# stochasticHydroTools/PSE

Measured on AMD Instinct MI355X. Metric: BD particle-steps/s (full PSE Brownian step: M.F + k-space noise + Lanczos M^1/2.psi + Euler), N=1e6, phi=0.1, higher is better.
Workload: dtype f64; 1 GPU; random-sphere suspension N=1000000, phi=0.1, cubic L=347.29, grid 256^3, xi=0.4405, rcut=5.966, P=6, error=0.001, kT=1.0, dt=0.001; parallelism=1 GPU

## Files before the change

include/pse_amd.h:

```cpp
#ifndef PSE_AMD_H
#define PSE_AMD_H

#ifdef __cplusplus
extern "C" {
#endif

typedef struct { double x, y, z, w; } pse_double4;
typedef struct { double x, y, z; } pse_double3;
typedef struct { int x, y, z; } pse_int3;

typedef struct pse_handle pse_handle;

enum pse_status {
    PSE_OK = 0,
    PSE_ERR_INVALID = -1,
    PSE_ERR_HIP = -2,
    PSE_ERR_FFT = -3,
    PSE_ERR_COMM = -4,
    PSE_ERR_NUMERIC = -5
};

typedef struct pse_params {
    unsigned int n_max;
    double Lx, Ly, Lz, xy;
// ... 241 lines not shown
int pse_angle_forces(pse_angles *a, const pse_double4 *pos, pse_double4 *force ,
                     int accumulate, double *out8 );

#define PSE_DIHEDRAL_HARMONIC 0
#define PSE_DIHEDRAL_OPLS     1
typedef struct pse_dihedrals pse_dihedrals;
int pse_dihedrals_create(pse_handle *h, unsigned n, unsigned ndihedrals,
                         const unsigned *quads_host ,
                         const unsigned *types_host ,
                         int ntypes, const int *kind_host , const double *params_host ,
                         pse_dihedrals **out);
int pse_dihedrals_destroy(pse_dihedrals *d);
int pse_dihedral_forces(pse_dihedrals *d, const pse_double4 *pos, pse_double4 *force ,
                        int accumulate, double *out8 );
int pse_debug_copy_grid(pse_handle *h, int stage, double *host_out);
int pse_debug_spread(pse_handle *h, const pse_double4 *pos, const pse_double4 *force, const unsigned int *group_members,
                     unsigned int N);
int pse_debug_gather(pse_handle *h, const pse_double4 *pos, const double *grid_host, const unsigned int *group_members,
                     unsigned int N, pse_double4 *vel_out);
int pse_debug_far_path(pse_handle *h, unsigned int N, int *out6);
int pse_debug_wave_grid(pse_handle *h, const double *grid_in_host, double xi, double eta, int noise, double kT, double dt,
                        unsigned int timestep, int poison, double *grid_out_host);
int pse_debug_fft_path(pse_handle *h, int *out8);
int pse_debug_kvector(pse_handle *h, int n, const int *ijk_host, double *out_host);
int pse_debug_grid_placement(pse_handle *h, int *tried, float *ms_first, float *ms_kept);
int pse_debug_vq_roundtrip(int n, const double *rows_host, double *out_host);
#define PSE_DEBUG_LZ_NSCAL 400
typedef struct pse_debug_lz_decision {
    int m_lo, m_hi, done_iters, have_last_beta, pending_beta, first, last, normalised, m_max;
    double tol, seq;
} pse_debug_lz_decision;
typedef struct pse_debug_lz_outcome {
    int done, m_final, checked, status;
    double stepnorm;
    double t_prev[104];
    double coef[104];
    double mirror[5];
} pse_debug_lz_outcome;
int pse_debug_lz_decide(const double *scal_host, int n_dec, const pse_debug_lz_decision *dec, double open0, pse_debug_lz_outcome *out);
int pse_debug_lz_decide_supported(int m_hi);
int pse_debug_matvec_ms(pse_handle *h, int reps, float *ms_per_launch);

typedef struct pse_team pse_team;
int pse_team_unique_id(void *id128_host);
int pse_team_create(pse_handle **members, int n_members, const void *id128_host, pse_team **out);
typedef struct pse_host_xfer {
// ... 77 lines not shown
```

pse_amd/_lib.py:

```python
import ctypes
import os

_HERE = os.path.dirname(os.path.abspath(__file__))


def asan_dir():
    d = os.environ.get("PSE_ASAN_DIR")
    if not d:
        return None
    if not os.path.exists(os.path.join(d, ".pse_asan_build")):
        import sys
        print(f"pse_amd: PSE_ASAN_DIR={d} ignored: no sanitizer build there (python -m pse_amd.build --asan writes one)", file=sys.stderr)
        return None
    if not getattr(asan_dir, "_said", False):
        import sys
        print(f"pse_amd: using the CPU SANITIZER build in {d} (PSE_ASAN_DIR): device entry points are stubs", file=sys.stderr)
        asan_dir._said = True
    return d


_ASAN_DIR = asan_dir()
LIB_PATH = os.path.join(_ASAN_DIR or _HERE, "libpse_amd.so")

PSE_OK = 0
# ... 155 lines not shown
    "pse_isf_store": (_i, [_vp, _i]),
    "pse_isf_correlate": (_i, [_vp, _i, _vp, _vp, _i, _vp, _vp]),
    "pse_host_rouse_weights": (_i, [_u, _i, _vp]),
    "pse_bonds_create": (_i, [_vp, _u, _u, _vp, _vp, _i, _vp, _vp, _vp, _vp]),
    "pse_bonds_destroy": (_i, [_vp]),
    "pse_bond_forces": (_i, [_vp, _vp, _vp, _i, _vp]),
    "pse_bonds_overstretched": (_i, [_vp, _vp]),
    "pse_host_bond_rows": (_i, [_u, _u, _vp, _vp, _vp, _vp]),
    "pse_angles_create": (_i, [_vp, _u, _u, _vp, _vp, _i, _vp, _vp, _vp, _vp]),
    "pse_angles_destroy": (_i, [_vp]),
    "pse_angle_forces": (_i, [_vp, _vp, _vp, _i, _vp]),
    "pse_host_angle_rows": (_i, [_u, _u, _vp, _vp, _vp, _vp]),
    "pse_dihedrals_create": (_i, [_vp, _u, _u, _vp, _vp, _i, _vp, _vp, _vp]),
    "pse_dihedrals_destroy": (_i, [_vp]),
    "pse_dihedral_forces": (_i, [_vp, _vp, _vp, _i, _vp]),
    "pse_host_dihedral_rows": (_i, [_u, _u, _vp, _vp, _vp, _vp]),
    "pse_eval_realspace": (_i, [_vp, _dp, _i, _dp, _dp]),
    "pse_debug_copy_grid": (_i, [_vp, _i, _dp]),
    "pse_debug_spread": (_i, [_vp, _vp, _vp, _vp, _u]),
    "pse_debug_gather": (_i, [_vp, _vp, _dp, _vp, _u, _vp]),
    "pse_debug_far_path": (_i, [_vp, _u, _ip]),
    "pse_debug_wave_grid": (_i, [_vp, _dp, _d, _d, _i, _d, _d, _u, _i, _dp]),
    "pse_debug_fft_path": (_i, [_vp, _ip]),
    "pse_debug_kvector": (_i, [_vp, _i, _ip, _dp]),
    "pse_debug_grid_placement": (_i, [_vp, _ip, ctypes.POINTER(ctypes.c_float), ctypes.POINTER(ctypes.c_float)]),
    "pse_debug_vq_roundtrip": (_i, [_i, _dp, _dp]),
    "pse_debug_lz_decide": (_i, [_dp, _i, ctypes.POINTER(pse_debug_lz_decision), _d, ctypes.POINTER(pse_debug_lz_outcome)]),
    "pse_debug_lz_decide_supported": (_i, [_i]),
    "pse_debug_matvec_ms": (_i, [_vp, _i, ctypes.POINTER(ctypes.c_float)]),
    "pse_team_unique_id": (_i, [_vp]),
    "pse_team_create": (_i, [ctypes.POINTER(_vp), _i, _vp, ctypes.POINTER(_vp)]),
    "pse_team_create_transport": (_i, [_vp, ctypes.POINTER(pse_transport), ctypes.POINTER(_vp)]),
    "pse_team_destroy": (_i, [_vp]),
    "pse_team_debug_solo": (_i, [_vp, _i]),
    "pse_team_mobility": (_i, [_vp, ctypes.POINTER(_vp), ctypes.POINTER(_vp), ctypes.POINTER(_vp), _vp, _u, _i]),
    "pse_team_brownian_velocity": (_i, [_vp, ctypes.POINTER(_vp), ctypes.POINTER(_vp), ctypes.POINTER(_vp), _vp, _u, _d, _d, _u, _ip]),
    "pse_team_step": (_i, [_vp, ctypes.POINTER(_vp), ctypes.POINTER(_vp), ctypes.POINTER(_vp), ctypes.POINTER(_vp),
                           ctypes.POINTER(_vp), _vp, _u, _d, _d, _u, _d, _ip]),
    "pse_team_step_local": (_i, [_vp, ctypes.POINTER(_vp), ctypes.POINTER(_vp), ctypes.POINTER(_vp), ctypes.POINTER(_vp),
                                 ctypes.POINTER(_vp), ctypes.POINTER(_vp), ctypes.POINTER(_vp), _d, _d, _u, _d, _i, _ip]),
    "pse_local_layout": (_i, [_vp, _ip, _ip, _ip, _ip, _ip]),
    "pse_team_local_status": (_i, [_vp, _ip]),
    "pse_team_set_lanczos_extra": (_i, [_vp, _i]),
    "pse_set_lanczos_extra": (_i, [_vp, _i]),
    "pse_set_lanczos_operator": (_i, [_vp, _i]),
    "pse_get_lanczos_operator": (_i, [_vp, _ip]),
# ... 41 lines not shown
```

pse_amd/csrc/asan_stub.cpp:

```cpp
#include <algorithm>
#include <cmath>
#include <cstdint>
#include <vector>

#include "pse_err.h"

using namespace pse;

struct Topology;
struct pse_handle {
    pse_params par;
    Derived d;
    pse_info info;
    std::vector<double> coef;
    int n_intervals = 0;
    unsigned long long steps = 0;
    int lz_op = PSE_LANCZOS_RECORDS16;
    std::vector<Topology *> topologies;
};
struct Topology {
    pse_handle *h;
    std::vector<int> row_off;
    std::vector<unsigned> entries;
    Topology(pse_handle *h, size_t noff, size_t nent) : h(h), row_off(noff), entries(nent) {}
// ... 422 lines not shown
    if (!force && !out8) return fail(PSE_ERR_INVALID, "pse_dihedral_forces: force and out8 are both null: nothing to compute");
    return 0;
}

int pse_set_stream(pse_handle *, void *) { return no_device("pse_set_stream"); }
int pse_set_timing(pse_handle *, int) { return no_device("pse_set_timing"); }
int pse_set_async(pse_handle *, int) { return no_device("pse_set_async"); }
int pse_set_timestep_offset(pse_handle *, const unsigned int *) { return no_device("pse_set_timestep_offset"); }
int pse_debug_last_gate(pse_handle *, int *) { return no_device("pse_debug_last_gate"); }
int pse_set_neighbor_skin(pse_handle *, double) { return no_device("pse_set_neighbor_skin"); }
int pse_neighbor_stats(pse_handle *, double *, unsigned long long *, unsigned long long *) { return no_device("pse_neighbor_stats"); }
int pse_mobility(pse_handle *, const pse_double4 *, const pse_double4 *, pse_double4 *, const unsigned int *, unsigned int, int) { return no_device("pse_mobility"); }
int pse_brownian_velocity(pse_handle *, const pse_double4 *, const pse_double4 *, pse_double4 *, const unsigned int *, unsigned int, double,
                          double, unsigned int, int *) { return no_device("pse_brownian_velocity"); }
int pse_sqrt_mreal(pse_handle *, const pse_double4 *, const pse_double4 *, pse_double4 *, const unsigned int *, unsigned int, double, int *) { return no_device("pse_sqrt_mreal"); }
int pse_random_psi(pse_handle *, pse_double4 *, const unsigned int *, unsigned int, unsigned int) { return no_device("pse_random_psi"); }
int pse_eval_realspace(pse_handle *, const double *, int, double *, double *) { return no_device("pse_eval_realspace"); }
int pse_debug_copy_grid(pse_handle *, int, double *) { return no_device("pse_debug_copy_grid"); }
int pse_debug_spread(pse_handle *, const pse_double4 *, const pse_double4 *, const unsigned int *, unsigned int) { return no_device("pse_debug_spread"); }
int pse_debug_gather(pse_handle *, const pse_double4 *, const double *, const unsigned int *, unsigned int, pse_double4 *) { return no_device("pse_debug_gather"); }
int pse_debug_far_path(pse_handle *, unsigned int, int *) { return no_device("pse_debug_far_path"); }
int pse_debug_wave_grid(pse_handle *, const double *, double, double, int, double, double, unsigned int, int, double *) { return no_device("pse_debug_wave_grid"); }
int pse_debug_fft_path(pse_handle *, int *) { return no_device("pse_debug_fft_path"); }
int pse_debug_kvector(pse_handle *, int, const int *, double *) { return no_device("pse_debug_kvector"); }
int pse_debug_grid_placement(pse_handle *, int *, float *, float *) { return no_device("pse_debug_grid_placement"); }
int pse_debug_vq_roundtrip(int, const double *, double *) { return no_device("pse_debug_vq_roundtrip"); }
int pse_debug_lz_decide(const double *, int, const pse_debug_lz_decision *, double, pse_debug_lz_outcome *) { return no_device("pse_debug_lz_decide"); }
int pse_debug_lz_decide_supported(int) { return 0; }
int pse_debug_matvec_ms(pse_handle *, int, float *) { return no_device("pse_debug_matvec_ms"); }
int pse_set_lanczos_extra(pse_handle *, int) { return no_device("pse_set_lanczos_extra"); }
int pse_set_lanczos_operator(pse_handle *h, int op) {
    if (!h) return fail(PSE_ERR_INVALID, "pse_set_lanczos_operator: null handle");
    if (op != PSE_LANCZOS_RECORDS16 && op != PSE_LANCZOS_FP64) return fail(PSE_ERR_INVALID, "pse_set_lanczos_operator: %d is not an operator", op);
    h->lz_op = op;
    return 0;
}
int pse_get_lanczos_operator(pse_handle *h, int *op) {
    if (!h || !op) return fail(PSE_ERR_INVALID, "pse_get_lanczos_operator: null argument");
    *op = h->lz_op;
    return 0;
}
int pse_brownian_velocity_part(pse_handle *, const pse_double4 *, const pse_double4 *, pse_double4 *, const unsigned int *, unsigned int, double,
                               double, unsigned int, int, int *) { return no_device("pse_brownian_velocity_part"); }
int pse_integrate(pse_handle *, pse_double4 *, const pse_double4 *, pse_double3 *, pse_int3 *, const pse_double4 *, const unsigned int *, unsigned int,
                  double, double) { return no_device("pse_integrate"); }
int pse_team_redistribute_local(pse_team *, pse_double4 *const *, pse_double4 *const *, pse_double3 *const *, pse_int3 *const *, pse_double4 *const *,
// ... 21 lines not shown
```

pse_amd/csrc/pse_capi.hip:

```cpp
#include <hip/hip_runtime.h>
#include <rccl/rccl.h>
#include <rocfft/rocfft.h>

#include <algorithm>
#include <chrono>
#include <cmath>
#include <cstdarg>
#include <cstdio>
#include <cstring>
#include <dlfcn.h>
#include <functional>
#include <future>
#include <memory>
#include <mutex>
#include <thread>
#include <string>
#include <vector>

#include "../../include/pse_amd.h"
#include "pse_err.h"
#include "pse_host.h"
#include "pse_kernels.h"
#include "pse_farfield.h"
#include "pse_fft.h"
// ... 791 lines not shown
    const double seq = (double)++h->lz_seq;
    h->lz_last_queued = true;
    int rg[3][2];
    const int nrg_all = update_ranges(h, N, rg);
    VecOut y = lz_y(h, false);
    auto vector_part = [&](int j, const int *gate) {
        launch_lz_update(lz_vec(h, j), y, lz_vec(h, j - 1), lz_vec(h, j + 1), j, h->scal, rg, nrg_all, h->stream,
                         nullptr, 0, h->sc_host_dev, gate, vq_of(h), h->lz_sums);
    };
    auto iteration = [&](int j, bool scalars_only, const int *gate) -> int {
        const bool have_y = j == 0 && h->w_is_mpsi;
        const bool fused = !have_y && h->nb.cap > 0 && h->nb_valid;
        if (!fused && !have_y) {
            if (gate) return fail(PSE_ERR_NUMERIC, "queued Lanczos: a gated iteration needs the pair list");
            TRY(lz_real_ok(h, j));
            TRY(real(T, j == 0 ? &pse_handle::psi_s : &pse_handle::V, &pse_handle::w_s, (size_t)j * h->n_pad, 0, N, true));
        }
        y = lz_y(h, fused);
        const double4 *vjm1 = lz_vec4(h, j - 1);
        const bool split = fused && j > 0;
        if (fused)
            launch_mreal_lanczos(h->pos_s, lz_vec(h, j), y, row_map(0, N), h->cell_off, h->dbox, h->nc, h->d.rcut, h->d.self, h->coef, h->nb,
                                 LzFuse{split ? nullptr : vjm1, h->partials, h->npart_cap, nullptr, nullptr, nullptr, h->lz_sums, lz_update_grid(N)}, h->scal, nullptr, nullptr, h->stream,
                                 h->vl_use ? h->vl : VerletList{}, split ? 4 : 1, gate, DevRowArgs{}, j > 0 ? vq_of(h) : nullptr);
        else if (!(j == 0 && h->sums0_done))
            launch_lz_dots(lz_vec4(h, j), h->w_s, vjm1, 0, N, h->partials, h->npart_cap, h->scal, h->stream);
        h->w_is_mpsi = false; h->sums0_done = false;
        if (scalars_only) launch_lz_update(lz_vec(h, j), y, lz_vec(h, j - 1), lz_vec(h, j + 1), j, h->scal, rg, 0, h->stream, nullptr, 0,
                                           h->sc_host_dev, gate);
        else vector_part(j, gate);
        return 0;
    };
    for (int j = 0; j < target; ++j) TRY(iteration(j, j == target - 1, nullptr));
    LzDecide d{};
    d.m_lo = std::max(m_in - 1, 1); d.m_hi = target; d.done_iters = target; d.first = 1; d.last = extra == 0 ? 1 : 0; d.m_max = M_MAX; d.tol = tol;
    launch_lz_decide(d, h->scal, h->lz_state, h->sc_host_dev, seq, h->stream);
    int done = target;
    for (int x = 0; x < extra; ++x) {
        vector_part(done - 1, stop);
        TRY(iteration(done, true, stop));
        d.m_lo = d.m_hi = done + 1; d.done_iters = done + 1; d.pending_beta = done; d.first = 0; d.last = x == extra - 1 ? 1 : 0;
        launch_lz_decide(d, h->scal, h->lz_state, h->sc_host_dev, seq, h->stream);
        ++done;
    }
    TRY(te(h, PH_LANCZOS));
    if (before_first_wait) TRY(before_first_wait());
    if (before_combine) TRY(before_combine());
// ... 28 lines not shown
                             h == h0 ? h->sc_host_dev : nullptr, nullptr, T.G <= 1 ? vq_of(h) : nullptr, T.G <= 1 ? h->lz_sums : nullptr);
        }
    };
    while (true) {
        for (; done < target; ++done) {
            const bool have_y = done == 0 && h0->w_is_mpsi;
            const bool fused = !have_y && h0->nb.cap > 0 && h0->nb_valid;
            const bool timed = done == 1 && fused;
            if (!fused && !have_y) {
                TRY(lz_real_ok(h0, done));
                TRY(real(T, done == 0 ? &pse_handle::psi_s : &pse_handle::V, &pse_handle::w_s, (size_t)done * h0->n_pad, 0, N, true));
            }
            y_from_list = fused;
            for (pse_handle *h : act(T)) {
                int lo, hi;
                row_range(h, N, lo, hi);
                const double4 *vjm1 = lz_vec4(h, done - 1);
                if (fused) {
                    const bool ev = timed && h->timing;
                    const bool split = done > 0 && T.G <= 1;
                    launch_mreal_lanczos(h->pos_s, lz_vec(h, done), lz_y(h, true), row_map(lo, hi), h->cell_off, h->dbox, h->nc, h->d.rcut, h->d.self, h->coef,
                                         h->nb, LzFuse{split ? nullptr : vjm1, h->partials, h->npart_cap, nullptr, nullptr, nullptr, h->lz_sums, lz_update_grid(N)}, h->scal,
                                         ev ? h->ph[PH_MATVEC].a : nullptr, ev ? h->ph[PH_MATVEC].b : nullptr, h->stream,
                                         h->vl_use ? h->vl : VerletList{}, split ? 4 : 1, nullptr, DevRowArgs{}, done > 0 && T.G <= 1 ? vq_of(h) : nullptr);
                    if (timed) h->matvec_timed = true;
                } else if (!(done == 0 && h->sums0_done)) {
                    launch_lz_dots(lz_vec4(h, done), h->w_s, vjm1, lo, hi, h->partials, h->npart_cap, h->scal, h->stream);
                }
                h->w_is_mpsi = false; h->sums0_done = false;
            }
            if (pump) TRY(pump->upto(n_exchanges));
            ++n_exchanges;
            TRY(team_lanczos_exchange(T, [](pse_handle *h) { return (double *)h->w_s; }));
            update(done, done == target - 1);
        }
        TRY(lz_wait_scalars(T, hook_done, before_first_wait));
        if (T.solo >= 0) { st.m_final = done; break; }
        LzDecide d{};
        d.first = pending_beta == 0; d.pending_beta = pending_beta;
        TRY(lz_decide_batch(d, m_in, done, tol, sc, st));
        if (st.done) break;
        update(done - 1, false);
        pending_beta = done;
        target = std::min(M_MAX, done + std::max(2, done / 4));
    }
    if (st.m_final == 0) {
        if (m_io) *m_io = m_in;
// ... 566 lines not shown
        e = hipStreamSynchronize(h->stream);
    }
    if (e == hipSuccess) e = hipMemcpy(f_host, buf + n, n * sizeof(double), hipMemcpyDeviceToHost);
    if (e == hipSuccess) e = hipMemcpy(g_host, buf + 2 * n, n * sizeof(double), hipMemcpyDeviceToHost);
    (void)hipFree(buf);
    if (e != hipSuccess) return fail(PSE_ERR_HIP, "pse_eval_realspace: %s", hipGetErrorString(e));
    return 0;
}

extern "C" int pse_debug_matvec_ms(pse_handle *h, int reps, float *ms_per_launch) {
    if (!h || !ms_per_launch || reps < 1) return fail(PSE_ERR_INVALID, "pse_debug_matvec_ms: bad argument");
    HIPCHK(hipSetDevice(h->device));
    if (h->n_slabs != 1 || !h->nb_valid || h->nb.cap <= 0 || h->sorted_N <= 0)
        return fail(PSE_ERR_INVALID, "pse_debug_matvec_ms: needs the pair list of a Brownian call on a single-GPU engine (call it right after one)");
    const int N = h->sorted_N;
    RowMap rm{};
    rm.n = 1; rm.lo[0] = 0; rm.hi[0] = N;
    hipEvent_t e0 = nullptr, e1 = nullptr;
    HIPCHK(hipEventCreate(&e0)); HIPCHK(hipEventCreate(&e1));
    auto run = [&](int n) {
        for (int r = 0; r < n; ++r)
            launch_mreal_lanczos(h->pos_s, lz_vec(h, 1), lz_y(h, true), rm, h->cell_off, h->dbox, h->nc, h->d.rcut, h->d.self, h->coef, h->nb,
                                 LzFuse{h->psi_s, h->partials, h->npart_cap, nullptr, nullptr, nullptr}, h->scal, nullptr, nullptr, h->stream,
                                 VerletList{}, 1, nullptr, DevRowArgs{}, vq_of(h), true);
    };
    run(2);
    HIPCHK(hipEventRecord(e0, h->stream));
    run(reps);
    HIPCHK(hipEventRecord(e1, h->stream));
    HIPCHK(hipEventSynchronize(e1));
    float ms = 0;
    HIPCHK(hipEventElapsedTime(&ms, e0, e1));
    (void)hipEventDestroy(e0); (void)hipEventDestroy(e1);
    HIPCHK(hipGetLastError());
    *ms_per_launch = ms / (float)reps;
    return 0;
}
extern "C" int pse_debug_vq_roundtrip(int n, const double *rows_host, double *out_host) {
    if (n < 0 || (n > 0 && (!rows_host || !out_host))) return fail(PSE_ERR_INVALID, "pse_debug_vq_roundtrip: null argument");
    if (n == 0) return 0;
    double *d_in = nullptr, *d_out = nullptr;
    hipError_t e = hipMalloc((void **)&d_in, (size_t)3 * n * sizeof(double));
    if (e == hipSuccess) e = hipMalloc((void **)&d_out, (size_t)3 * n * sizeof(double));
    if (e == hipSuccess) e = hipMemcpy(d_in, rows_host, (size_t)3 * n * sizeof(double), hipMemcpyHostToDevice);
    if (e == hipSuccess) { launch_vq_roundtrip(d_in, d_out, n, nullptr); e = hipGetLastError(); }
    if (e == hipSuccess) e = hipMemcpy(out_host, d_out, (size_t)3 * n * sizeof(double), hipMemcpyDeviceToHost);
    (void)hipFree(d_in); (void)hipFree(d_out);
// ... 123 lines not shown
        if (grid_in_host) HIPCHK(hipMemcpyAsync(dst, grid_in_host + (size_t)c * plane * G.nxl, plane * G.nxl * sizeof(double), hipMemcpyHostToDevice, h->wstream));
        else HIPCHK(hipMemsetAsync(dst, 0, plane * G.nxl * sizeof(double), h->wstream));
    }
    WaveArgs a{0, noise != 0, kT, dt, timestep};
    a.xi = xi; a.eta = eta;
    TRY(wave_forward_transforms(h, 1));
    TRY(wave_compute(T, a, 1));
    TRY(wave_compute(T, a, 2));
    HIPCHK(hipGetLastError());
    HIPCHK(hipStreamSynchronize(h->wstream));
    for (int c = 0; c < 3; ++c)
        HIPCHK(hipMemcpy(grid_out_host + (size_t)c * plane * G.nxl, h->rgrid + c * nr + plane * G.hl, plane * G.nxl * sizeof(double),
                         hipMemcpyDeviceToHost));
    return 0;
}

extern "C" int pse_debug_fft_path(pse_handle *h, int *out8) {
    if (!h || !out8) return fail(PSE_ERR_INVALID, "pse_debug_fft_path: null argument");
    const FftChoice none{FFT_ROCFFT, 0};
    const FftChoice x = h->xfuse ? xfft_choice(h->G, scale_args(h, false, 0.0, 1.0, 0)) : none;
    const FftChoice y = h->own_y ? yfft_choice(h->G, h->tun.yfft_kb) : none;
    const int out[8] = {h->xfuse, h->own_y, h->own_z, x.kernel, x.kb, y.kernel, y.kb, h->own_z ? zfft_choice(h->G.Nz) : FFT_ROCFFT};
    std::copy(out, out + 8, out8);
    return 0;
}

extern "C" int pse_debug_copy_grid(pse_handle *h, int stage, double *host_out) {
    if (!h || !host_out) return fail(PSE_ERR_INVALID, "bad argument");
    (void)stage;
    HIPCHK(hipSetDevice(h->device));
    HIPCHK(hipStreamSynchronize(h->stream));
    if (h->side) HIPCHK(hipStreamSynchronize(h->side));
    const size_t plane = (size_t)h->G.Ny * h->G.Nz, full = plane * (h->G.nxl + h->G.hl + h->G.nhalo);
    for (int c = 0; c < 3; ++c)
        HIPCHK(hipMemcpy(host_out + (size_t)c * plane * h->G.nxl, h->rgrid + c * full + plane * h->G.hl, plane * h->G.nxl * sizeof(double),
                         hipMemcpyDeviceToHost));
    return 0;
}

extern "C" int pse_team_unique_id(void *id128_host) {
    if (!id128_host) return fail(PSE_ERR_INVALID, "null argument");
    static_assert(sizeof(ncclUniqueId) == 128, "RCCL unique id is 128 bytes");
    ncclUniqueId id;
    NCCLCHK(ncclGetUniqueId(&id));
    memcpy(id128_host, &id, sizeof id);
    return 0;
// ... 337 lines not shown
```

pse_amd/csrc/pse_engine.hip:

```cpp
#include <hip/hip_runtime.h>
#include <rocfft/rocfft.h>

#include <algorithm>
#include <cmath>
#include <cstdio>
#include <cstring>
#include <mutex>
#include <string>
#include <vector>

#include "pse_forces.h"
#include "pse_handle.h"

static std::once_flag g_fft_once;

static int set_lanczos_op(pse_handle *h, int op) {
    if (op == PSE_LANCZOS_FP64 && h->nb.cap > 0 && !h->nb64) {
        HIPCHK(hipSetDevice(h->device));
        TRY(dmalloc(h, &h->nb64, nb_list64_bytes((size_t)h->n_pad + 1024, h->nb.cap) / sizeof(double4)));
        h->info.device_bytes = h->bytes;
    }
    if (op != h->lz_op) h->nb_valid = false;
    h->lz_op = op;
    h->nb.c64 = op == PSE_LANCZOS_FP64 ? h->nb64 : nullptr;
// ... 212 lines not shown
    set_dbox(h);
    h->n_slabs = std::max(1, p->n_slabs);
    h->loc.on = p->local_rows != 0;
    if (h->loc.on && h->n_slabs < 2) return fail(PSE_ERR_INVALID, "local_rows needs n_slabs >= 2 (an owned-particle rank is a member of a team)");
    roctx_lookup();
    {
        auto ienv = [](const char *name, int dflt) { const char *v = getenv(name); return v ? atoi(v) : dflt; };
        auto &t = h->tun;
        t.cell_bz = std::min(16, std::max(0, ienv("PSE_CELL_BZ", 6)));
        if (const char *v = getenv("PSE_SKIN")) t.skin = atof(v);
        t.overlap = ienv("PSE_OVERLAP", 1);
        t.no_xfuse = getenv("PSE_NO_XFUSE") != nullptr;
        t.own_y = ienv("PSE_OWN_Y", 1); t.own_y_pow2 = ienv("PSE_OWN_Y_POW2", 1); t.yfft_kb = ienv("PSE_YFFT_KB", 4); t.own_z = ienv("PSE_OWN_Z", 1); t.yslab_regs = ienv("PSE_YSLAB_REGS", 1);
        if (const char *v = getenv("PSE_WAVE_MODE")) t.wave_mode = !strcmp(v, "slab") ? 1 : (!strcmp(v, "replicated") ? 2 : 0);
        t.spread_tz = ienv("PSE_SPREAD_TZ", 0); t.spread_nw = ienv("PSE_SPREAD_NW", 0);
        t.gather_bz = ienv("PSE_GATHER_BZ", 0); t.xmix_runtime = ienv("PSE_XMIX", 0) == 1; t.xfft_small_wide = ienv("PSE_XFFT_SMALL_KB", 2) == 8;
        t.verbose = ienv("PSE_VERBOSE", 0) > 0;
        t.team_sstep = ienv("PSE_TEAM_SSTEP", 1) > 0;
        t.lz_extra = std::max(0, std::min(32, ienv("PSE_LANCZOS_EXTRA", 2)));
        t.place_trials = std::max(0, std::min(12, ienv("PSE_PLACE_TRIALS", 10)));
        t.vq = ienv("PSE_VQ", 1);
        if (const char *v = getenv("PSE_LANCZOS_OP")) t.lz_op = !strcmp(v, "fp64") ? PSE_LANCZOS_FP64 : PSE_LANCZOS_RECORDS16;
        t.rows24 = ienv("PSE_ROWS24", 1);
        if (const char *v = getenv("PSE_TEAM_SCHED")) {
            int a = 1, b = 2, c = 3;
            if (sscanf(v, "%d,%d,%d", &a, &b, &c) == 3) { t.team_sched[0] = a; t.team_sched[1] = b; t.team_sched[2] = c; }
        }
        h->sw.force_tz = t.spread_tz; h->sw.force_nw = t.spread_nw; h->sw.force_bz = t.gather_bz;
    }
    {
        double skin = h->tun.skin;
        const int nint = (int)std::ceil(d.rcut * RS_PER_UNIT) + 1;
        const double gam = std::max(std::fabs(p->xy), p->max_strain);
        const double wmin = std::min(std::min(h->box.Lx / std::sqrt(1.0 + gam * gam), h->box.Ly), h->box.Lz);
        if (!(skin > 0.0) || h->n_slabs > 1 || !mreal_table_in_lds(nint * 2 * RS_NCOEF) || d.rcut + skin > 0.5 * wmin)
            skin = 0.0;
        h->skin = h->skin_max = skin;
    }
    TRY(set_cells(h, std::max(std::fabs(p->xy), p->max_strain)));
    fill_info(d, &h->info);
    h->info.ncell_x = h->nc.nx; h->info.ncell_y = h->nc.ny; h->info.ncell_z = h->nc.nz;

    DGrid &G = h->G;
    G.Nx = d.Nx; G.Ny = d.Ny; G.Nz = d.Nz; G.Nzh = d.Nz / 2 + 1; G.P = d.P;
    G.Nzp = (G.Nzh + 7) & ~7;
    h->n_slabs = std::max(1, p->n_slabs);
// ... 310 lines not shown
```

pse_amd/csrc/pse_handle.h:

```cpp
#pragma once
#include <hip/hip_runtime.h>
#include <rocfft/rocfft.h>

#include <type_traits>
#include <vector>

#include "../../include/pse_amd.h"
#include "pse_err.h"
#include "pse_host.h"
#include "pse_kernels.h"
#include "pse_farfield.h"
#include "pse_fft.h"
#include "pse_vectors.h"
#include "pse_local.h"

using namespace pse;

#define HIPCHK(x)                                                                                      \
    do {                                                                                               \
        hipError_t e_ = (x);                                                                           \
        if (e_ != hipSuccess) return fail(PSE_ERR_HIP, "%s failed: %s (%s:%d)", #x, hipGetErrorString(e_), __FILE__, __LINE__); \
    } while (0)
#define TRY(x)              \
    do {                    \
// ... 120 lines not shown
    struct Tuning {
        int cell_bz = 6;
        double skin = 0.4;
        int overlap = 1;
        bool no_xfuse = false;
        int own_y_pow2 = 1;
        int own_y = 1;
        int own_z = 1;
        int yslab_regs = 1;
        int yfft_kb = 4;
        int wave_mode = 0;
        int spread_tz = 0, spread_nw = 0;
        int gather_bz = 0;
        int xmix_runtime = 0;
        int xfft_small_wide = 0;
        bool verbose = false;
        bool team_sstep = true;
        int team_sched[3] = {1, 2, 3};
        int vq = 1;
        int place_trials = 10;
        int lz_extra = 2;
        int lz_op = PSE_LANCZOS_RECORDS16;
        int rows24 = 1;
    } tun;
    DCells bidx_nc = {0, 0, 0};
    hipEvent_t ev_fork = nullptr, ev_join = nullptr;
    bool overlap_all = false;
    bool side_on = false;
    hipEvent_t ev_scal = nullptr;
    int n_max = 0, n_pad = 0;
    unsigned *keys = nullptr, *keys_s = nullptr, *vals = nullptr, *perm = nullptr, *tag_s = nullptr;
    void *sort_tmp = nullptr;
    int *cell_cnt = nullptr;
    size_t sort_tmp_bytes = 0;
    int *cell_off = nullptr;
    double *pv_rows = nullptr;
    std::vector<DeviceObject *> topologies;
    DeviceArrays arrays;
    FftPlans fft;
    PinnedBuffers pinned;
    Streams streams;
    Events events;
    int *cnt_block = nullptr;
    size_t cnt_bins = 0;
    SpreadWork sw = {};
    NbList nb = {};
// ... 135 lines not shown
```

pse_amd/csrc/pse_kernels.h:

```cpp
#pragma once
#include <hip/hip_runtime.h>
#include <stdint.h>

#include "pse_device.h"

namespace pse {

size_t cell_sort_temp_bytes(size_t ncell);
struct CellRanges {
    int n, c0[3], c1[3];
    __device__ __forceinline__ bool cell(int c) const {
        if (n == 0) return true;
        for (int q = 0; q < n; ++q) if (c >= c0[q] && c < c1[q]) return true;
        return false;
    }
    __device__ __forceinline__ bool row(int s, const int *__restrict__ cell_off) const {
        if (n == 0) return true;
        for (int q = 0; q < n; ++q) if (s >= cell_off[c0[q]] && s < cell_off[c1[q]]) return true;
        return false;
    }
};
struct RowMap {
    int n, lo[3], hi[3], base[3];
    __host__ __device__ int list_rows() const { return n ? base[n - 1] + ((hi[n - 1] - lo[n - 1] + 255) & ~255) : 0; }
// ... 95 lines not shown
    int npart_cap;
    const double4 *q, *p, *u;
    const double *upd;
    int n_upd;
};
enum { LZG_QW1 = 0, LZG_W1W1, LZG_W1W2, LZG_W2W2, LZG_PW1, LZG_PW2, LZG_UW2, LZG_QQ, LZ_NGRAM };
void launch_mreal(const double4 *pos_s, const float4 *posf_s, const double4 *vec_s, double4 *out_s, RowMap rows,
                  const int *cell_off, DBox box, DCells nc, double rcut, double self, const double *coef, int ncoef, NbList nb,
                  int mode, hipStream_t s, const double4 *vec2_s = nullptr, double4 *out2_s = nullptr,
                  VerletList vl = VerletList{}, int vl_mode = VL_NONE,
                  const double2 *pv = nullptr,
                  double *sums0 = nullptr, int sums0_cap = 0, double *scal = nullptr,
                  Gate gate = Gate{},
                  DevRowArgs dr = DevRowArgs{});
bool mreal_table_in_lds(int ncoef);
void launch_mreal_lanczos(const double4 *pos_s, VecIn vec, VecOut out, RowMap rows, const int *cell_off,
                          DBox box, DCells nc, double rcut, double self, const double *coef, NbList nb, LzFuse lz,
                          double *scal, hipEvent_t ev_begin, hipEvent_t ev_end, hipStream_t s,
                          VerletList vl = VerletList{},
                          int sums = 1,
                          const int *stop = nullptr,
                          DevRowArgs dr = DevRowArgs{},
                          const void *vec_q = nullptr,
                          bool no_reduce = false);
int mreal_partials_needed(int rows);
void launch_eval_fg(const double *r, int n, const double *coef, double *f, double *g, hipStream_t s);

}
```

pse_amd/csrc/pse_kernels.hip:

```cpp
#include "pse_kernels.h"
#include "pse_vectors.h"
#include "pse_farbin.h"

#include <hipcub/hipcub.hpp>

namespace pse {

constexpr unsigned KEY_FOREIGN = 0xFFFFFFFFu;
__global__ void k_cell_keys(const double4 *__restrict__ pos, const unsigned *__restrict__ group, int N, DBox box,
                            DCells nc, unsigned *__restrict__ keys, unsigned *__restrict__ rank, int *__restrict__ cnt, CellRanges need,
                            SlabBook sb, Gate gate) {
    if (gate.closed()) return;
    const int g = blockIdx.x * blockDim.x + threadIdx.x;
    const bool live = g < N;
    unsigned key = 0;
    bool mine = false;
    if (live) {
        const unsigned idx = group ? group[g] : (unsigned)g;
        const double4 p = pos[idx];
        double fx, fy, fz;
        frac_coords(box, p.x, p.y, p.z, fx, fy, fz);
        const int cx = cell_coord(fx, nc.nx), cy = cell_coord(fy, nc.ny), cz = cell_coord(fz, nc.nz);
        const int zb = cz / nc.bz;
        key = (unsigned)cell_slot(nc, cx, cy, zb, cz - zb * nc.bz);
// ... 555 lines not shown
    if (TWO) out2_s[i] = make_double4(wx, wy, wz, 0.0);
    if (LIST) nb.cnt[i] = total > nb.cap ? -1 : total;
}

__device__ __forceinline__ void eval_fg_lean(double r2, const double *__restrict__ coef, double &f, double &gmf_r2) {
    const double ir = rsqrt(r2), r = r2 * ir, ir2 = ir * ir;
    double f0, g0;
    if (r > 2.0) { const double ir3 = ir * ir2; f0 = 0.75 * ir + 0.5 * ir3; g0 = 1.5 * ir - ir3; }
    else { f0 = 1.0 - 0.28125 * r; g0 = 1.0 - 0.1875 * r; }
    const double s = r * RS_PER_UNIT;
    const int k = (int)s;
    const double t = 2.0 * (s - k) - 1.0;
    const double *c = coef + (size_t)k * (2 * RS_NCOEF);
    double fw = c[RS_DEG], gw = c[RS_NCOEF + RS_DEG];
#pragma unroll 1
    for (int q = RS_DEG - 1; q >= 0; --q) {
        fw = fma(fw, t, c[q]);
        gw = fma(gw, t, c[RS_NCOEF + q]);
    }
    f = f0 - fw;
    gmf_r2 = ((g0 - gw) - f) * ir2;
}

template <int FUSE, int UNROLL, int NT, int WSP = 1, bool VQ = false, bool F64 = false>
__global__ void __launch_bounds__(NT, (WSP == 4 ? 5 : 1))
k_mreal_list(const double4 *__restrict__ pos_s, const double4 *__restrict__ vec_s, double4 *__restrict__ out_s, RowMap rm_arg,
             DBox box, double self, NbList nb, LzFuse lz,
             const int *__restrict__ cell_off, DCells nc, double rcut2, const double *__restrict__ coef, VerletList vl,
             const int *__restrict__ stop, DevRowArgs dr, const vq4 *__restrict__ vec_q = nullptr, int packed = 0) {
    if (stop && *stop) return;
    const VecIn vin{reinterpret_cast<const double *>(vec_s), packed & 1};
    const VecOut vout{reinterpret_cast<double *>(out_s), (packed >> 1) & 1};
    const RowMapRegs rm(rm_arg, dr.rm);
    int nb_live = gridDim.x;
    if (dr.rm) {
        nb_live = (rm.list_rows() + (WSP > 1 ? 64 : NT) - 1) / (WSP > 1 ? 64 : NT);
        if ((int)blockIdx.x >= nb_live) {
            if (FUSE && threadIdx.x == 0)
                for (int t = 0; t < (FUSE == 2 || FUSE == 3 ? (int)LZ_NGRAM : 3); ++t) lz.partials[(size_t)t * lz.npart_cap + blockIdx.x] = 0.0;
            return;
        }
    }
    __shared__ double sh[4];
    static_assert(WSP == 1 || NT == 64 * WSP, "split rows: one wave per slot phase");
    const int wv = WSP > 1 ? (int)(threadIdx.x >> 6) : 0;
    const int lr = WSP > 1 ? xcd_block(blockIdx.x, nb_live) * 64 + (int)(threadIdx.x & 63)
                           : xcd_block(blockIdx.x, nb_live) * NT + (int)threadIdx.x;
    const int i = rm.row(lr);
    const bool active = i >= 0;
    double ux = 0.0, uy = 0.0, uz = 0.0;
    double4 vi = make_double4(0.0, 0.0, 0.0, 0.0);
    if (active) {
        row_load(vin, i, vi.x, vi.y, vi.z);
        const int cnt = nb.cnt[i];
        if (cnt >= 0) {
            if (wv == 0) { ux = self * vi.x; uy = self * vi.y; uz = self * vi.z; }
            const int lane = lr & 63;
            const char *rec = nb.data + (size_t)(lr >> 6) * nb.cap * NB_REC;
            static_assert(UNROLL == 4, "one list group per iteration");
            for (int s0 = UNROLL * wv; s0 < cnt; s0 += UNROLL * WSP) {
                const char *grp = rec + (size_t)(s0 >> 2) * (4 * NB_REC);
                unsigned e[UNROLL];
                nb4 c[UNROLL];
                d4v c64[F64 ? UNROLL : 1];
#pragma unroll
                for (int u = 0; u < UNROLL; ++u) {
                    c[u] = __builtin_nontemporal_load((const nb4 *)grp + u * 64 + lane);
                    if (F64) c64[u] = __builtin_nontemporal_load((const d4v *)nb.c64 + (size_t)(lr >> 6) * nb.cap * 64 + (size_t)(s0 >> 2) * 256 + u * 64 + lane);
                    e[u] = c[u].x;
                    if (u && s0 + u >= cnt) e[u] = e[0];
                }
                double2 vxy[UNROLL];
                double vz[UNROLL];
                vq4 vq[UNROLL];
#pragma unroll
                for (int u = 0; u < UNROLL; ++u) {
                    if (VQ && !F64) { vq[u] = vec_q[e[u] & JMASK]; continue; }
                    if (vin.packed) { row24_load(vin.p, e[u] & JMASK, vxy[u].x, vxy[u].y, vz[u]); continue; }
// ... 39 lines not shown
            const double4 pi = pos_s[i];
            ux = self * vi.x; uy = self * vi.y; uz = self * vi.z;
            double fx, fy, fz;
            frac_coords(box, pi.x, pi.y, pi.z, fx, fy, fz);
            const int cx = cell_coord(fx, nc.nx), cy = cell_coord(fy, nc.ny), cz = cell_coord(fz, nc.nz);
            for_each_run(nc, cell_off, cx, cy, cz, [&](int jb, int je, unsigned) {
                for (int j = jb; j < je; ++j) {
                    const double4 pj = pos_s[j];
                    double dx = pi.x - pj.x, dy = pi.y - pj.y, dz = pi.z - pj.z;
                    min_image(box, dx, dy, dz);
                    const double r2 = dx * dx + dy * dy + dz * dz;
                    if (r2 < rcut2 && j != i && r2 > 0.0) {
                        double f, h;
                        eval_fg_lean(r2, coef, f, h);
                        double3 Fj;
                        row_load(vin, j, Fj.x, Fj.y, Fj.z);
                        if (F64) pair_apply64(pair_coef64(f, h, dx, dy, dz), Fj.x, Fj.y, Fj.z, ux, uy, uz);
                        else pair_apply(pair_coef(f, h, dx, dy, dz), Fj.x, Fj.y, Fj.z, ux, uy, uz);
                    }
                }
            });
        }
    }
    if (WSP > 1) {
        __shared__ double red[WSP > 1 ? (WSP - 1) * 3 * 64 : 1];
        const int ln = threadIdx.x & 63;
        if (wv > 0) { red[((wv - 1) * 3 + 0) * 64 + ln] = ux; red[((wv - 1) * 3 + 1) * 64 + ln] = uy; red[((wv - 1) * 3 + 2) * 64 + ln] = uz; }
        __syncthreads();
        if (wv > 0) return;
        for (int w = 0; w < WSP - 1; ++w) { ux += red[(w * 3 + 0) * 64 + ln]; uy += red[(w * 3 + 1) * 64 + ln]; uz += red[(w * 3 + 2) * 64 + ln]; }
    }
    if (FUSE == 2 || FUSE == 3) {
        double g[LZ_NGRAM];
#pragma unroll
        for (int t = 0; t < LZ_NGRAM; ++t) g[t] = 0.0;
        if (active) {
            auto dot = [](const double4 &x, double yx, double yy, double yz) { return x.x * yx + x.y * yy + x.z * yz; };
            const double4 z4 = make_double4(0.0, 0.0, 0.0, 0.0);
            const double4 p = lz.p ? lz.p[i] : z4;
            if (FUSE == 2) {
                const double4 q = lz.q[i], u = lz.u ? lz.u[i] : z4;
                g[LZG_QW1] = dot(q, vi.x, vi.y, vi.z); g[LZG_W1W1] = dot(vi, vi.x, vi.y, vi.z); g[LZG_W1W2] = dot(vi, ux, uy, uz);
                g[LZG_W2W2] = ux * ux + uy * uy + uz * uz; g[LZG_PW1] = dot(p, vi.x, vi.y, vi.z);
                g[LZG_PW2] = dot(p, ux, uy, uz); g[LZG_UW2] = dot(u, ux, uy, uz); g[LZG_QQ] = dot(q, q.x, q.y, q.z);
            } else {
                g[LZG_QW1] = dot(vi, ux, uy, uz); g[LZG_W1W1] = ux * ux + uy * uy + uz * uz; g[LZG_PW1] = dot(p, ux, uy, uz);
// ... 76 lines not shown
#define PSE_CELLS(L, C, T, V) do { if ((L) && f64) PSE_CELLS_F(L, C, T, V, (L)); else PSE_CELLS_F(L, C, T, V, false); } while (0)
#define PSE_CELLS_PK(L, T, D) do { if ((L) && f64) PSE_CELLS_PK_F(L, T, D, (L)); else PSE_CELLS_PK_F(L, T, D, false); } while (0)
    if (dr.rm) {
        if (list && two) PSE_CELLS_PK(true, true, true); else PSE_CELLS_PK(false, false, true);
        return;
    }
    if (pv && cl && !wr && vl_mode != VL_USE && (two || !list)) {
        if (list) PSE_CELLS_PK(true, true, false); else PSE_CELLS_PK(false, false, false);
    } else if (list) {
        if (cl && two) { if (wr) PSE_CELLS(true, true, true, true); else PSE_CELLS(true, true, true, false); }
        else if (cl) { if (wr) PSE_CELLS(true, true, false, true); else PSE_CELLS(true, true, false, false); }
        else PSE_CELLS(true, false, false, false);
    } else if (cl) { if (wr) PSE_CELLS(false, true, false, true); else PSE_CELLS(false, true, false, false); }
    else PSE_CELLS(false, false, false, false);
#undef PSE_CELLS_PK
#undef PSE_CELLS
#undef PSE_CELLS_PK_F
#undef PSE_CELLS_F
    if (sums0 && list && two && cl)
        launch_lz_reduce(sums0, (int)g.x * (TPB / 64), sums0_cap, 3, scal, nullptr, s);
}

int mreal_partials_needed(int rows) { return nblocks(std::max(rows, 1), 64); }
void launch_mreal_lanczos(const double4 *pos_s, VecIn vec, VecOut out, RowMap rm, const int *cell_off,
                          DBox box, DCells nc, double rcut, double self, const double *coef, NbList nb, LzFuse lz,
                          double *scal, hipEvent_t ev_begin, hipEvent_t ev_end, hipStream_t s, VerletList vl,
                          int sums, const int *stop, DevRowArgs dr, const void *vec_q, bool no_reduce) {
    const double4 *vec_s = reinterpret_cast<const double4 *>(vec.p);
    double4 *w = reinterpret_cast<double4 *>(out.p);
    const int packed = (vec.packed ? 1 : 0) | (out.packed ? 2 : 0);
    const int rows = std::max(dr.rm ? dr.rows_cap : rm.list_rows(), 1);
    if (ev_begin) (void)hipEventRecord(ev_begin, s);
    const int nb64 = nblocks(rows, 64);
#define PSE_LIST(F) hipLaunchKernelGGL((k_mreal_list<F, 4, 256, 4>), dim3(nb64), dim3(256), 0, s, pos_s, vec_s, w, rm, box, self, nb, lz, cell_off, nc, rcut * rcut, coef, vl, stop, dr, nullptr, packed)
#define PSE_LIST64(F) hipLaunchKernelGGL((k_mreal_list<F, 4, 256, 4, false, true>), dim3(nb64), dim3(256), 0, s, pos_s, vec_s, w, rm, box, self, nb, lz, cell_off, nc, rcut * rcut, coef, vl, stop, dr, nullptr, packed)
    if (nb.c64) {
        if (sums == 0) PSE_LIST64(0); else if (sums == 1) PSE_LIST64(1); else if (sums == 2) PSE_LIST64(2); else if (sums == 3) PSE_LIST64(3); else PSE_LIST64(4);
    } else if (sums == 1 && vec_q)
        hipLaunchKernelGGL((k_mreal_list<1, 4, 256, 4, true>), dim3(nb64), dim3(256), 0, s, pos_s, vec_s, w, rm, box, self, nb, lz, cell_off, nc, rcut * rcut, coef, vl, stop, dr,
                           (const vq4 *)vec_q, packed);
    else if (sums == 4 && vec_q)
        hipLaunchKernelGGL((k_mreal_list<4, 4, 256, 4, true>), dim3(nb64), dim3(256), 0, s, pos_s, vec_s, w, rm, box, self, nb, lz, cell_off, nc, rcut * rcut, coef, vl, stop, dr,
                           (const vq4 *)vec_q, packed);
    else if (sums == 0) PSE_LIST(0); else if (sums == 1) PSE_LIST(1); else if (sums == 2) PSE_LIST(2); else if (sums == 3) PSE_LIST(3); else PSE_LIST(4);
#undef PSE_LIST64
#undef PSE_LIST
    if (ev_end) (void)hipEventRecord(ev_end, s);
    if (no_reduce) return;
    if (sums == 4) launch_lz_reduce_split(lz.partials + lz.npart_cap, nb64, lz.upd, lz.n_upd, scal, stop, s);
    else if (sums >= 1) launch_lz_reduce(lz.partials, nb64, lz.npart_cap, sums == 1 ? 3 : (int)LZ_NGRAM, scal, stop, s);
}

__global__ void k_eval_fg(const double *__restrict__ r, int n, const double *__restrict__ coef, double *f, double *g) {
    const int i = blockIdx.x * blockDim.x + threadIdx.x;
    if (i >= n) return;
    double ff, h;
    const double r2 = r[i] * r[i];
    eval_fg(r2, coef, ff, h);
    f[i] = ff;
    g[i] = ff + h * r2;
}
void launch_eval_fg(const double *r, int n, const double *coef, double *f, double *g, hipStream_t s) {
    hipLaunchKernelGGL(k_eval_fg, dim3(nblocks(n, TPB)), dim3(TPB), 0, s, r, n, coef, f, g);
}

}
```

pse_amd/engine.py:

```python
import ctypes
import math

from . import _lib
from ._lib import pse_info, pse_params


def _ptr(t):
    return ctypes.c_void_p(t.data_ptr()) if t is not None else None


def _is_cuda(t, *dtypes):
    import torch
    return isinstance(t, torch.Tensor) and t.is_cuda and t.dtype in dtypes and t.is_contiguous()


def _chk4(t, name, n=None):
    import torch
    if not (_is_cuda(t, torch.float64) and t.dim() == 2 and t.shape[1] == 4):
        raise ValueError(f"{name} must be a contiguous (N,4) float64 CUDA tensor")
    if n is not None and t.shape[0] < n:
        raise ValueError(f"{name} has fewer than {n} rows")


def _chk_group(g, name="group"):
# ... 1260 lines not shown
        _lib.check(self._lib.pse_debug_gather(self._h, _ptr(pos), grid.ctypes.data_as(ctypes.POINTER(ctypes.c_double)), _ptr(group), n,
                                              _ptr(vel)))
        return vel

    FAR_PATH_FIELDS = ("spread_fast", "TZ", "NW", "gather_fast", "BZ", "shear")

    def far_path(self, n):
        out = (ctypes.c_int * 6)()
        _lib.check(self._lib.pse_debug_far_path(self._h, int(n), out))
        return dict(zip(self.FAR_PATH_FIELDS, out))

    FFT_PATH_FIELDS = ("xfuse", "own_y", "own_z", "x", "x_kb", "y", "y_kb", "z")
    FFT_X_KERNELS = ("rocfft+k_scale", "k_xfft_scale", "k_xfft_scale_cols", "k_xfft_scale_mixed/ct", "k_xfft_scale_mixed/rt")
    FFT_Y_KERNELS = ("rocfft", "k_fft_cols/ct", "k_fft_cols/rt", "k_yfft_regs")
    FFT_Z_KERNELS = ("rocfft", "k_zfft_rows", "k_zfft_rows_g")

    def fft_path(self):
        out = (ctypes.c_int * 8)()
        _lib.check(self._lib.pse_debug_fft_path(self._h, out))
        d = dict(zip(self.FFT_PATH_FIELDS, out))
        d["x"] = self.FFT_X_KERNELS[d["x"]]; d["y"] = self.FFT_Y_KERNELS[d["y"]]; d["z"] = self.FFT_Z_KERNELS[d["z"]]
        return d

    def debug_wave_grid(self, grid=None, xi=0.0, eta=0.0, noise=False, kT=0.0, dt=1.0, timestep=0, poison=True):
        import numpy as np
        i = self.info()
        shape = (3, i["Nx"] // max(1, self.params.n_slabs), i["Ny"], i["Nz"])
        dp = ctypes.POINTER(ctypes.c_double)
        src = None
        if grid is not None:
            grid = np.ascontiguousarray(grid, dtype=np.float64)
            if grid.shape != shape:
                raise ValueError(f"grid must have the shape of debug_grid(), not {grid.shape}")
            src = grid.ctypes.data_as(dp)
        out = np.zeros(shape)
        _lib.check(self._lib.pse_debug_wave_grid(self._h, src, float(xi), float(eta), int(bool(noise)), float(kT), float(dt), int(timestep),
                                                 int(bool(poison)), out.ctypes.data_as(dp)))
        return out

    def debug_kvector(self, ijk):
        import numpy as np
        ijk = np.ascontiguousarray(ijk, dtype=np.int32)
        out = np.zeros((len(ijk), 5))
        _lib.check(self._lib.pse_debug_kvector(self._h, len(ijk), ijk.ctypes.data_as(ctypes.POINTER(ctypes.c_int)),
                                               out.ctypes.data_as(ctypes.POINTER(ctypes.c_double))))
        return out
# ... 183 lines not shown
```

Baseline: 337.2 million particle-steps/s.

## Prefetch neighbor-list records into LDS via async global_load_lds in Lanczos matvec

Measured after the change: 339.8 million particle-steps/s (median of 6 runs). No clear change (+0.8%).

```diff
diff --git a/include/pse_amd.h b/include/pse_amd.h
--- a/include/pse_amd.h
+++ b/include/pse_amd.h
@@ -287,6 +287,7 @@
 int pse_debug_wave_grid(pse_handle *h, const double *grid_in_host, double xi, double eta, int noise, double kT, double dt,
                         unsigned int timestep, int poison, double *grid_out_host);
 int pse_debug_fft_path(pse_handle *h, int *out8);
+int pse_debug_matvec_path(pse_handle *h, int *out4);
 int pse_debug_kvector(pse_handle *h, int n, const int *ijk_host, double *out_host);
 int pse_debug_grid_placement(pse_handle *h, int *tried, float *ms_first, float *ms_kept);
 int pse_debug_vq_roundtrip(int n, const double *rows_host, double *out_host);
diff --git a/pse_amd/_lib.py b/pse_amd/_lib.py
--- a/pse_amd/_lib.py
+++ b/pse_amd/_lib.py
@@ -201,6 +201,7 @@
     "pse_debug_far_path": (_i, [_vp, _u, _ip]),
     "pse_debug_wave_grid": (_i, [_vp, _dp, _d, _d, _i, _d, _d, _u, _i, _dp]),
     "pse_debug_fft_path": (_i, [_vp, _ip]),
+    "pse_debug_matvec_path": (_i, [_vp, _ip]),
     "pse_debug_kvector": (_i, [_vp, _i, _ip, _dp]),
     "pse_debug_grid_placement": (_i, [_vp, _ip, ctypes.POINTER(ctypes.c_float), ctypes.POINTER(ctypes.c_float)]),
     "pse_debug_vq_roundtrip": (_i, [_i, _dp, _dp]),
diff --git a/pse_amd/csrc/asan_stub.cpp b/pse_amd/csrc/asan_stub.cpp
--- a/pse_amd/csrc/asan_stub.cpp
+++ b/pse_amd/csrc/asan_stub.cpp
@@ -468,6 +468,7 @@
 int pse_debug_far_path(pse_handle *, unsigned int, int *) { return no_device("pse_debug_far_path"); }
 int pse_debug_wave_grid(pse_handle *, const double *, double, double, int, double, double, unsigned int, int, double *) { return no_device("pse_debug_wave_grid"); }
 int pse_debug_fft_path(pse_handle *, int *) { return no_device("pse_debug_fft_path"); }
+int pse_debug_matvec_path(pse_handle *, int *) { return no_device("pse_debug_matvec_path"); }
 int pse_debug_kvector(pse_handle *, int, const int *, double *) { return no_device("pse_debug_kvector"); }
 int pse_debug_grid_placement(pse_handle *, int *, float *, float *) { return no_device("pse_debug_grid_placement"); }
 int pse_debug_vq_roundtrip(int, const double *, double *) { return no_device("pse_debug_vq_roundtrip"); }
diff --git a/pse_amd/csrc/pse_capi.hip b/pse_amd/csrc/pse_capi.hip
--- a/pse_amd/csrc/pse_capi.hip
+++ b/pse_amd/csrc/pse_capi.hip
@@ -837,7 +837,7 @@
         if (fused)
             launch_mreal_lanczos(h->pos_s, lz_vec(h, j), y, row_map(0, N), h->cell_off, h->dbox, h->nc, h->d.rcut, h->d.self, h->coef, h->nb,
                                  LzFuse{split ? nullptr : vjm1, h->partials, h->npart_cap, nullptr, nullptr, nullptr, h->lz_sums, lz_update_grid(N)}, h->scal, nullptr, nullptr, h->stream,
-                                 h->vl_use ? h->vl : VerletList{}, split ? 4 : 1, gate, DevRowArgs{}, j > 0 ? vq_of(h) : nullptr);
+                                 h->vl_use ? h->vl : VerletList{}, split ? 4 : 1, gate, DevRowArgs{}, j > 0 ? vq_of(h) : nullptr, false, h->tun.list_prefetch);
         else if (!(j == 0 && h->sums0_done))
             launch_lz_dots(lz_vec4(h, j), h->w_s, vjm1, 0, N, h->partials, h->npart_cap, h->scal, h->stream);
         h->w_is_mpsi = false; h->sums0_done = false;
@@ -912,7 +912,7 @@
                     launch_mreal_lanczos(h->pos_s, lz_vec(h, done), lz_y(h, true), row_map(lo, hi), h->cell_off, h->dbox, h->nc, h->d.rcut, h->d.self, h->coef,
                                          h->nb, LzFuse{split ? nullptr : vjm1, h->partials, h->npart_cap, nullptr, nullptr, nullptr, h->lz_sums, lz_update_grid(N)}, h->scal,
                                          ev ? h->ph[PH_MATVEC].a : nullptr, ev ? h->ph[PH_MATVEC].b : nullptr, h->stream,
-                                         h->vl_use ? h->vl : VerletList{}, split ? 4 : 1, nullptr, DevRowArgs{}, done > 0 && T.G <= 1 ? vq_of(h) : nullptr);
+                                         h->vl_use ? h->vl : VerletList{}, split ? 4 : 1, nullptr, DevRowArgs{}, done > 0 && T.G <= 1 ? vq_of(h) : nullptr, false, h->tun.list_prefetch);
                     if (timed) h->matvec_timed = true;
                 } else if (!(done == 0 && h->sums0_done)) {
                     launch_lz_dots(lz_vec4(h, done), h->w_s, vjm1, lo, hi, h->partials, h->npart_cap, h->scal, h->stream);
@@ -1525,7 +1525,7 @@
         for (int r = 0; r < n; ++r)
             launch_mreal_lanczos(h->pos_s, lz_vec(h, 1), lz_y(h, true), rm, h->cell_off, h->dbox, h->nc, h->d.rcut, h->d.self, h->coef, h->nb,
                                  LzFuse{h->psi_s, h->partials, h->npart_cap, nullptr, nullptr, nullptr}, h->scal, nullptr, nullptr, h->stream,
-                                 VerletList{}, 1, nullptr, DevRowArgs{}, vq_of(h), true);
+                                 VerletList{}, 1, nullptr, DevRowArgs{}, vq_of(h), true, h->tun.list_prefetch);
     };
     run(2);
     HIPCHK(hipEventRecord(e0, h->stream));
@@ -1695,6 +1695,14 @@
     const FftChoice y = h->own_y ? yfft_choice(h->G, h->tun.yfft_kb) : none;
     const int out[8] = {h->xfuse, h->own_y, h->own_z, x.kernel, x.kb, y.kernel, y.kb, h->own_z ? zfft_choice(h->G.Nz) : FFT_ROCFFT};
     std::copy(out, out + 8, out8);
+    return 0;
+}
+
+extern "C" int pse_debug_matvec_path(pse_handle *h, int *out4) {
+    if (!h || !out4) return fail(PSE_ERR_INVALID, "pse_debug_matvec_path: null argument");
+    const MatvecPath p = h->nb.cap > 0 ? mreal_lanczos_path(h->nb, vq_of(h), 1, DevRowArgs{}, h->tun.list_prefetch) : MatvecPath{h->nb.c64 != nullptr, false, false};
+    const int out[4] = {p.fp64 ? 1 : 0, p.mirror ? 1 : 0, h->rows24 ? 1 : 0, p.prefetch ? 1 : 0};
+    std::copy(out, out + 4, out4);
     return 0;
 }
 
diff --git a/pse_amd/csrc/pse_engine.hip b/pse_amd/csrc/pse_engine.hip
--- a/pse_amd/csrc/pse_engine.hip
+++ b/pse_amd/csrc/pse_engine.hip
@@ -258,6 +258,7 @@
         t.vq = ienv("PSE_VQ", 1);
         if (const char *v = getenv("PSE_LANCZOS_OP")) t.lz_op = !strcmp(v, "fp64") ? PSE_LANCZOS_FP64 : PSE_LANCZOS_RECORDS16;
         t.rows24 = ienv("PSE_ROWS24", 1);
+        t.list_prefetch = ienv("PSE_LIST_PREFETCH", 1);
         if (const char *v = getenv("PSE_TEAM_SCHED")) {
             int a = 1, b = 2, c = 3;
             if (sscanf(v, "%d,%d,%d", &a, &b, &c) == 3) { t.team_sched[0] = a; t.team_sched[1] = b; t.team_sched[2] = c; }
diff --git a/pse_amd/csrc/pse_handle.h b/pse_amd/csrc/pse_handle.h
--- a/pse_amd/csrc/pse_handle.h
+++ b/pse_amd/csrc/pse_handle.h
@@ -166,6 +166,7 @@
         int lz_extra = 2;
         int lz_op = PSE_LANCZOS_RECORDS16;
         int rows24 = 1;
+        int list_prefetch = 1;
     } tun;
     DCells bidx_nc = {0, 0, 0};
     hipEvent_t ev_fork = nullptr, ev_join = nullptr;
diff --git a/pse_amd/csrc/pse_kernels.h b/pse_amd/csrc/pse_kernels.h
--- a/pse_amd/csrc/pse_kernels.h
+++ b/pse_amd/csrc/pse_kernels.h
@@ -141,7 +141,10 @@
                           const int *stop = nullptr,
                           DevRowArgs dr = DevRowArgs{},
                           const void *vec_q = nullptr,
-                          bool no_reduce = false);
+                          bool no_reduce = false,
+                          bool prefetch = false);
+struct MatvecPath { bool fp64, mirror, prefetch; };
+MatvecPath mreal_lanczos_path(const NbList &nb, const void *vec_q, int sums, const DevRowArgs &dr, bool prefetch);
 int mreal_partials_needed(int rows);
 void launch_eval_fg(const double *r, int n, const double *coef, double *f, double *g, hipStream_t s);
 
diff --git a/pse_amd/csrc/pse_kernels.hip b/pse_amd/csrc/pse_kernels.hip
--- a/pse_amd/csrc/pse_kernels.hip
+++ b/pse_amd/csrc/pse_kernels.hip
@@ -601,7 +601,15 @@
     gmf_r2 = ((g0 - gw) - f) * ir2;
 }
 
-template <int FUSE, int UNROLL, int NT, int WSP = 1, bool VQ = false, bool F64 = false>
+typedef __attribute__((address_space(3))) void lds_void_t;
+typedef __attribute__((address_space(1))) const void glb_void_t;
+template <int AUX>
+__device__ __forceinline__ void list_group_dma(const char *grp, int lane, nb4 *buf) {
+#pragma unroll
+    for (int u = 0; u < 4; ++u)
+        __builtin_amdgcn_global_load_lds((glb_void_t *)(grp + u * NB_REC + lane * 16), (lds_void_t *)(buf + u * 64), 16, 0, AUX);
+}
+template <int FUSE, int UNROLL, int NT, int WSP = 1, bool VQ = false, bool F64 = false, bool PF = false>
 __global__ void __launch_bounds__(NT, (WSP == 4 ? 5 : 1))
 k_mreal_list(const double4 *__restrict__ pos_s, const double4 *__restrict__ vec_s, double4 *__restrict__ out_s, RowMap rm_arg,
              DBox box, double self, NbList nb, LzFuse lz,
@@ -629,10 +637,44 @@
     const bool active = i >= 0;
     double ux = 0.0, uy = 0.0, uz = 0.0;
     double4 vi = make_double4(0.0, 0.0, 0.0, 0.0);
+    static_assert(!PF || (WSP == 4 && VQ && !F64 && UNROLL == 4), "the prefetching form: the split records kernel with the mirror");
+    constexpr int PF_AUX = 2;
+    __shared__ __attribute__((aligned(16))) nb4 pf_buf[PF ? WSP * UNROLL * 64 : 1];
+    nb4 *const wbuf = pf_buf + (PF ? wv * UNROLL * 64 : 0);
+    if (PF && active && wv < nb.cap / 4)
+        list_group_dma<PF_AUX>(nb.data + (size_t)(lr >> 6) * nb.cap * NB_REC + (size_t)wv * (4 * NB_REC), lr & 63, wbuf);
     if (active) {
         row_load(vin, i, vi.x, vi.y, vi.z);
         const int cnt = nb.cnt[i];
-        if (cnt >= 0) {
+        if (cnt >= 0 && PF) {
+            if (wv == 0) { ux = self * vi.x; uy = self * vi.y; uz = self * vi.z; }
+            const int lane = lr & 63;
+            const char *rec = nb.data + (size_t)(lr >> 6) * nb.cap * NB_REC;
+            for (int s0 = UNROLL * wv; s0 < cnt; s0 += UNROLL * WSP) {
+                asm volatile("s_waitcnt vmcnt(0)" ::: "memory");
+                nb4 c[UNROLL];
+#pragma unroll
+                for (int u = 0; u < UNROLL; ++u) c[u] = wbuf[u * 64 + lane];
+                asm volatile("s_waitcnt lgkmcnt(0)" : "+v"(c[0]), "+v"(c[1]), "+v"(c[2]), "+v"(c[3]) : : "memory");
+                __builtin_amdgcn_sched_barrier(0);
+                if (s0 + UNROLL * WSP < cnt) list_group_dma<PF_AUX>(rec + (size_t)((s0 >> 2) + WSP) * (4 * NB_REC), lane, wbuf);
+                unsigned e[UNROLL];
+                vq4 vq[UNROLL];
+#pragma unroll
+                for (int u = 0; u < UNROLL; ++u) {
+                    e[u] = c[u].x;
+                    if (u && s0 + u >= cnt) e[u] = e[0];
+                    vq[u] = vec_q[e[u] & JMASK];
+                }
+#pragma unroll
+                for (int u = 0; u < UNROLL; ++u) {
+                    const PairCoef pc = nb_unpack(c[u], s0 + u < cnt);
+                    double vx, vy, vz;
+                    vq_unpack(vq[u], vx, vy, vz);
+                    pair_apply(pc, vx, vy, vz, ux, uy, uz);
+                }
+            }
+        } else if (cnt >= 0) {
             if (wv == 0) { ux = self * vi.x; uy = self * vi.y; uz = self * vi.z; }
             const int lane = lr & 63;
             const char *rec = nb.data + (size_t)(lr >> 6) * nb.cap * NB_REC;
@@ -718,6 +760,7 @@
             });
         }
     }
+    if (PF) asm volatile("s_waitcnt vmcnt(0)" ::: "memory");
     if (WSP > 1) {
         __shared__ double red[WSP > 1 ? (WSP - 1) * 3 * 64 : 1];
         const int ln = threadIdx.x & 63;
@@ -840,10 +883,17 @@
 }
 
 int mreal_partials_needed(int rows) { return nblocks(std::max(rows, 1), 64); }
+MatvecPath mreal_lanczos_path(const NbList &nb, const void *vec_q, int sums, const DevRowArgs &dr, bool prefetch) {
+    MatvecPath p;
+    p.fp64 = nb.c64 != nullptr;
+    p.mirror = !p.fp64 && vec_q != nullptr && (sums == 1 || sums == 4);
+    p.prefetch = p.mirror && prefetch && !dr.rm;
+    return p;
+}
 void launch_mreal_lanczos(const double4 *pos_s, VecIn vec, VecOut out, RowMap rm, const int *cell_off,
                           DBox box, DCells nc, double rcut, double self, const double *coef, NbList nb, LzFuse lz,
                           double *scal, hipEvent_t ev_begin, hipEvent_t ev_end, hipStream_t s, VerletList vl,
-                          int sums, const int *stop, DevRowArgs dr, const void *vec_q, bool no_reduce) {
+                          int sums, const int *stop, DevRowArgs dr, const void *vec_q, bool no_reduce, bool prefetch) {
     const double4 *vec_s = reinterpret_cast<const double4 *>(vec.p);
     double4 *w = reinterpret_cast<double4 *>(out.p);
     const int packed = (vec.packed ? 1 : 0) | (out.packed ? 2 : 0);
@@ -852,7 +902,11 @@
     const int nb64 = nblocks(rows, 64);
 #define PSE_LIST(F) hipLaunchKernelGGL((k_mreal_list<F, 4, 256, 4>), dim3(nb64), dim3(256), 0, s, pos_s, vec_s, w, rm, box, self, nb, lz, cell_off, nc, rcut * rcut, coef, vl, stop, dr, nullptr, packed)
 #define PSE_LIST64(F) hipLaunchKernelGGL((k_mreal_list<F, 4, 256, 4, false, true>), dim3(nb64), dim3(256), 0, s, pos_s, vec_s, w, rm, box, self, nb, lz, cell_off, nc, rcut * rcut, coef, vl, stop, dr, nullptr, packed)
-    if (nb.c64) {
+#define PSE_LIST_PF(F) hipLaunchKernelGGL((k_mreal_list<F, 4, 256, 4, true, false, true>), dim3(nb64), dim3(256), 0, s, pos_s, vec_s, w, rm, box, self, nb, lz, cell_off, nc, rcut * rcut, coef, vl, stop, dr, (const vq4 *)vec_q, packed)
+    const MatvecPath path = mreal_lanczos_path(nb, vec_q, sums, dr, prefetch);
+    if (path.prefetch) {
+        if (sums == 1) PSE_LIST_PF(1); else PSE_LIST_PF(4);
+    } else if (nb.c64) {
         if (sums == 0) PSE_LIST64(0); else if (sums == 1) PSE_LIST64(1); else if (sums == 2) PSE_LIST64(2); else if (sums == 3) PSE_LIST64(3); else PSE_LIST64(4);
     } else if (sums == 1 && vec_q)
         hipLaunchKernelGGL((k_mreal_list<1, 4, 256, 4, true>), dim3(nb64), dim3(256), 0, s, pos_s, vec_s, w, rm, box, self, nb, lz, cell_off, nc, rcut * rcut, coef, vl, stop, dr,
@@ -861,6 +915,7 @@
         hipLaunchKernelGGL((k_mreal_list<4, 4, 256, 4, true>), dim3(nb64), dim3(256), 0, s, pos_s, vec_s, w, rm, box, self, nb, lz, cell_off, nc, rcut * rcut, coef, vl, stop, dr,
                            (const vq4 *)vec_q, packed);
     else if (sums == 0) PSE_LIST(0); else if (sums == 1) PSE_LIST(1); else if (sums == 2) PSE_LIST(2); else if (sums == 3) PSE_LIST(3); else PSE_LIST(4);
+#undef PSE_LIST_PF
 #undef PSE_LIST64
 #undef PSE_LIST
     if (ev_end) (void)hipEventRecord(ev_end, s);
diff --git a/pse_amd/engine.py b/pse_amd/engine.py
--- a/pse_amd/engine.py
+++ b/pse_amd/engine.py
@@ -1306,6 +1306,13 @@
         d["x"] = self.FFT_X_KERNELS[d["x"]]; d["y"] = self.FFT_Y_KERNELS[d["y"]]; d["z"] = self.FFT_Z_KERNELS[d["z"]]
         return d
 
+    MATVEC_PATH_FIELDS = ("fp64", "mirror", "rows24", "prefetch")
+
+    def matvec_path(self):
+        out = (ctypes.c_int * 4)()
+        _lib.check(self._lib.pse_debug_matvec_path(self._h, out))
+        return {k: bool(v) for k, v in zip(self.MATVEC_PATH_FIELDS, out)}
+
     def debug_wave_grid(self, grid=None, xi=0.0, eta=0.0, noise=False, kT=0.0, dt=1.0, timestep=0, poison=True):
         import numpy as np
         i = self.info()
```
